# yoshitomo-matsubara/sc2-benchmark

Hardware: AMD Instinct MI355X
Metric: images/s + bpp, Entropic-Student ResNet-50 224^2 (higher is better)
Workload: dtype bf16

## Files before the change

### sc2-benchmark_amd/csrc/conv1x1_kres.hip

```cpp
#include <stdlib.h>

#include <atomic>

#include <type_traits>

#include "sc2_common.h"

#ifndef SC2_NT_KRES
#define SC2_NT_KRES 0
#endif

namespace {

typedef __attribute__((address_space(3))) void *lds_ptr_t;
typedef float f32x2_t __attribute__((ext_vector_type(2)));
typedef __bf16 bf16x2_t __attribute__((ext_vector_type(2)));
__device__ __forceinline__ uint32_t pack2(f32x2_t v) {
    return __builtin_bit_cast(uint32_t, __builtin_convertvector(v, bf16x2_t));
}

#if defined(__HIP_DEVICE_COMPILE__)
typedef __amdgpu_buffer_rsrc_t buf_rsrc_t;
__device__ __forceinline__ buf_rsrc_t make_rsrc(const uint16_t *base, uint32_t bytes) {
    return __builtin_amdgcn_make_buffer_rsrc(const_cast<uint16_t *>(base), 0, (int)bytes, 0x00020000);
}
__device__ __forceinline__ void buf_load_lds16(buf_rsrc_t r, lds_ptr_t dst, uint32_t voff, uint32_t soff) {
    __builtin_amdgcn_raw_ptr_buffer_load_lds(r, dst, 16, (int)voff, (int)soff, 0, 0);
}
#else
typedef int buf_rsrc_t;
__device__ __forceinline__ buf_rsrc_t make_rsrc(const uint16_t *, uint32_t) { return 0; }
__device__ __forceinline__ void buf_load_lds16(buf_rsrc_t, lds_ptr_t, uint32_t, uint32_t) {}
#endif

__device__ __forceinline__ uint4 lds_read16(uint32_t addr) {
    uint4 v;
    asm volatile("ds_read_b128 %0, %1" : "=v"(v) : "v"(addr) : "memory");
    return v;
}

struct KresArgs {
    const uint16_t *__restrict__ x;
    const uint16_t *__restrict__ w;
    const float *__restrict__ bias;
    uint16_t *__restrict__ y;
    int M, Cout, relu, n_chunks, n_tiles;
    int H, W, OW, OHW, stride;
    unsigned in_bytes;
    unsigned *unit_ctr;
};

template <int K_, int BM_, int BNC_>
struct KresShape {
    static constexpr int K = K_, BM = BM_, BNC = BNC_;
    static constexpr int KS = K / 32, KSH = KS / 2;
    static constexpr int MT = BM / 16, NTW = BNC / 32;
    static constexpr int NB = MT * NTW, NOWN = NB / 2;
    static constexpr int A_BYTES = BM * K * 2;
    static constexpr int PPR = K * 2 / 1024;
    static constexpr int PIECES = A_BYTES / 1024, PIECES_PER_WAVE = PIECES / 4;
    static constexpr int XCH_OFF = 2 * A_BYTES;
    static constexpr int OIMG_OFF = XCH_OFF;
    static constexpr int LDS_BYTES = XCH_OFF + 16 * 1024;
    static constexpr int OUT_CHUNKS = BM * BNC * 2 / 16;
    static constexpr int STORES = OUT_CHUNKS >= 256 ? OUT_CHUNKS / 256 : 1;
    static_assert(A_BYTES == 65536 && (K / 64) * (BNC / 32) * 4 == 256, "64 KB A tile, 256 weight registers per wave");
    static_assert(4 * NOWN * 1024 <= 16 * 1024 && BM * BNC * 2 <= 16 * 1024 && STORES >= 1, "exchange / image area");
    static_assert(LDS_BYTES + 64 <= 160 * 1024, "one workgroup per CU");
};

template <class S>
__global__ __launch_bounds__(256, 1) void conv1x1_kres_kernel(const KresArgs p) {
    constexpr int K = S::K, BM = S::BM, BNC = S::BNC, KS = S::KS, KSH = S::KSH, MT = S::MT, NTW = S::NTW, NOWN = S::NOWN;
    extern __shared__ __attribute__((aligned(16))) unsigned char smem[];
    __shared__ int next_slot;
    const uint32_t lds_base = (uint32_t)(uintptr_t)(lds_ptr_t)smem;
    const int tid = threadIdx.x;
    const int lane = tid & 63;
    const int wave = __builtin_amdgcn_readfirstlane(tid >> 6);
    const int kh = wave >> 1, nh = wave & 1;
    const int frow = lane & 15, fq = lane >> 4;

    const int xcd = blockIdx.x & 7;
    const int j_x = blockIdx.x >> 3;
    const int chunk = j_x % p.n_chunks;
    const int wg_l = j_x / p.n_chunks;
    const int wgs_x = ((int)gridDim.x - xcd + 7) >> 3;
    const int wgs_c = (wgs_x - chunk + p.n_chunks - 1) / p.n_chunks;
    const int n_local = (p.n_tiles - xcd + 7) >> 3;
    unsigned *const my_ctr = p.unit_ctr + xcd * 16 + chunk;

    uint4 wreg[KSH][NTW];
    {
        const uint4 *wf = reinterpret_cast<const uint4 *>(p.w) + lane;
#pragma unroll
        for (int j = 0; j < NTW; ++j)
#pragma unroll
            for (int s = 0; s < KSH; ++s)
                wreg[s][j] = wf[((long long)(chunk * (BNC / 16) + nh * NTW + j) * KS + kh * KSH + s) * 64];
    }

    const buf_rsrc_t rs = make_rsrc(p.x, p.in_bytes);
    auto row_offsets = [&](int tile) -> uint32_t {
        const int m = (xcd + 8 * tile) * BM + (lane & (BM - 1));
        const bool ok = tile < n_local && m < p.M;
        long long pix = m;
        if (p.stride == 2) {
            const int mm = ok ? m : 0;
            const int im = mm / p.OHW, rem = mm - im * p.OHW;
            const int oh = rem / p.OW, ow = rem - oh * p.OW;
            pix = ((long long)im * p.H + 2 * oh) * p.W + 2 * ow;
        }
        return ok ? (uint32_t)(pix * (K * 2)) : 0xFFFFFFFFu;
    };
    auto issue_piece = [&](uint32_t rowoff_v, int buf, int k) {
        const int pc = wave + 4 * k;
        const int row = pc / S::PPR, part = pc % S::PPR;
        const uint32_t ro = (uint32_t)__builtin_amdgcn_readlane((int)rowoff_v, row);
        const bool ok = ro != 0xFFFFFFFFu;
        const uint32_t vo = ok ? (uint32_t)(((64 * part + lane) ^ (row & 15)) * 16) : 0x80000000u;
        buf_load_lds16(rs, (lds_ptr_t)(smem + buf * S::A_BYTES + pc * 1024), vo, ok ? ro : 0u);
    };

    int unit = wg_l;
    int next_unit = unit + wgs_c;
    {
        const uint32_t ro = row_offsets(unit);
#pragma unroll
        for (int k = 0; k < S::PIECES_PER_WAVE; ++k) issue_piece(ro, 0, k);
    }
    int g = 0;

    while (unit < n_local) {
        const int m0 = (xcd + 8 * unit) * BM;
        if (g != 0) asm volatile("s_waitcnt vmcnt(%0)" ::"n"(S::STORES) : "memory");
        else asm volatile("s_waitcnt vmcnt(0)" ::: "memory");
        __syncthreads();
        unsigned claimed = 0;
        if (tid == 0) {
            const unsigned one = 1u;
            asm volatile("global_atomic_add %0, %1, %2, off sc0" : "=v"(claimed) : "v"(my_ctr), "v"(one) : "memory");
        }
        const uint32_t ro_next = row_offsets(next_unit);
        const uint32_t ab = lds_base + (uint32_t)((g & 1) * S::A_BYTES);
        const uint32_t a_lane = ab + (uint32_t)(frow * (K * 2));
        f32x4_t acc[MT][NTW];
#pragma unroll
        for (int i = 0; i < MT; ++i)
#pragma unroll
            for (int j = 0; j < NTW; ++j) acc[i][j] = f32x4_t{0.f, 0.f, 0.f, 0.f};
        uint4 av[2][MT];
        {
            int fqo = fq;
            asm volatile("" : "+v"(fqo));
            const int ks = kh * KSH;
#pragma unroll
            for (int i = 0; i < MT; ++i)
                av[0][i] = lds_read16(a_lane + (uint32_t)(i * 16 * K * 2) + (uint32_t)((((ks * 4 + fqo) ^ frow)) << 4));
        }
        constexpr int PIECE_STEPS = 8;
        constexpr int PER_STEP = S::PIECES_PER_WAVE / PIECE_STEPS;
#pragma unroll
        for (int s = 0; s < KSH; ++s) {
            asm volatile("s_waitcnt lgkmcnt(0)" ::: "memory");
            __builtin_amdgcn_sched_barrier(0);
            if (s + 1 < KSH) {
                int fqo = fq;
                asm volatile("" : "+v"(fqo));
                const int ks = kh * KSH + s + 1;
#pragma unroll
                for (int i = 0; i < MT; ++i)
                    av[(s + 1) & 1][i] = lds_read16(a_lane + (uint32_t)(i * 16 * K * 2) + (uint32_t)((((ks * 4 + fqo) ^ frow)) << 4));
            }
#pragma unroll
            for (int i = 0; i < MT; ++i) {
                const bf16x8_t af = __builtin_bit_cast(bf16x8_t, av[s & 1][i]);
#pragma unroll
                for (int j = 0; j < NTW; ++j)
                    acc[i][j] = __builtin_amdgcn_mfma_f32_16x16x32_bf16(__builtin_bit_cast(bf16x8_t, wreg[s][j]), af, acc[i][j], 0, 0, 0);
            }
            __builtin_amdgcn_sched_barrier(0);
            if (s < PIECE_STEPS) {
#pragma unroll
                for (int q = 0; q < PER_STEP; ++q) issue_piece(ro_next, (g + 1) & 1, PER_STEP * s + q);
            }
        }
#pragma unroll
        for (int b = 0; b < NOWN; ++b) {
            const f32x4_t v = kh ? acc[b / NTW][b % NTW] : acc[(NOWN + b) / NTW][(NOWN + b) % NTW];
            *reinterpret_cast<f32x4_t *>(smem + S::XCH_OFF + ((wave * NOWN + b) * 64 + lane) * 16) = v;
        }
        __syncthreads();
        f32x4_t own[NOWN];
#pragma unroll
        for (int b = 0; b < NOWN; ++b) {
            const f32x4_t mine = kh ? acc[(NOWN + b) / NTW][(NOWN + b) % NTW] : acc[b / NTW][b % NTW];
            own[b] = mine + *reinterpret_cast<const f32x4_t *>(smem + S::XCH_OFF + (((wave ^ 2) * NOWN + b) * 64 + lane) * 16);
        }
        __syncthreads();
        {
            unsigned char *oimg = smem + S::OIMG_OFF;
            constexpr int CPI = BNC / 8;
            auto finish = [&](auto relu_c) {
                constexpr bool RELU = decltype(relu_c)::value;
#pragma unroll
                for (int b = 0; b < NOWN; ++b) {
                    const int bb = kh * NOWN + b;
                    const int i = bb / NTW, j = bb % NTW;
                    const int px = i * 16 + frow;
                    const int ch = nh * (BNC / 2) + j * 16 + fq * 4;
                    const float4 bias4 = *reinterpret_cast<const float4 *>(p.bias + chunk * BNC + ch);
                    f32x2_t v01 = f32x2_t{own[b][0], own[b][1]} + f32x2_t{bias4.x, bias4.y};
                    f32x2_t v23 = f32x2_t{own[b][2], own[b][3]} + f32x2_t{bias4.z, bias4.w};
                    if (RELU) {
                        v01 = f32x2_t{fmaxf(v01[0], 0.f), fmaxf(v01[1], 0.f)};
                        v23 = f32x2_t{fmaxf(v23[0], 0.f), fmaxf(v23[1], 0.f)};
                    }
                    uint2 o;
                    o.x = pack2(v01);
                    o.y = pack2(v23);
                    const int c = ch >> 3;
                    *reinterpret_cast<uint2 *>(oimg + px * (BNC * 2) + ((c ^ (px & (CPI - 1))) << 4) + (ch & 7) * 2) = o;
                }
            };
            if (p.relu) finish(std::true_type{});
            else finish(std::false_type{});
        }
        __syncthreads();
        {
            const unsigned char *oimg = smem + S::OIMG_OFF;
            uint4 *yo = reinterpret_cast<uint4 *>(p.y + (long long)chunk * BNC);
            constexpr int CPI = BNC / 8;
#pragma unroll
            for (int k = 0; k < S::STORES; ++k) {
                const int q = (tid + 256 * k) % S::OUT_CHUNKS;
                int row = q / CPI;
                const int c = q % CPI;
                row = m0 + row < p.M ? row : 0;
                const uint4 ov = *reinterpret_cast<const uint4 *>(oimg + row * (BNC * 2) + ((c ^ (row & (CPI - 1))) << 4));
                if (SC2_NT_KRES) sc2_store16_nt(yo + (long long)(m0 + row) * (p.Cout / 8) + c, ov);
                else yo[(long long)(m0 + row) * (p.Cout / 8) + c] = ov;
            }
        }
        if (tid == 0) {
            asm volatile("s_waitcnt vmcnt(%1)" : "+v"(claimed) : "n"(S::STORES) : "memory");
            next_slot = (int)(claimed + 2 * wgs_c);
            if (claimed == (unsigned)(n_local - 1)) *my_ctr = 0u;
        }
        __syncthreads();
        ++g;
        unit = next_unit;
        next_unit = __builtin_amdgcn_readfirstlane(next_slot);
    }
    asm volatile("s_waitcnt vmcnt(0)" ::: "memory");
}

constexpr int kRingK = 1024;
sc2_counter_ring g_ring_k;
std::atomic<unsigned> g_seq_k{0};

template <class S>
int launch_kres(KresArgs a, hipStream_t s) {
    a.n_chunks = a.Cout / S::BNC;
    a.n_tiles = (a.M + S::BM - 1) / S::BM;
    static bool attr_set_dev[SC2_MAX_DEVICES] = {};
    bool &attr_set = attr_set_dev[sc2_device_slot()];
    if (!attr_set) {
        (void)hipFuncSetAttribute(reinterpret_cast<const void *>(&conv1x1_kres_kernel<S>), hipFuncAttributeMaxDynamicSharedMemorySize,
                                  S::LDS_BYTES);
        attr_set = true;
    }
    const int g_cus_k = sc2_device_cus();
    unsigned *slot = g_ring_k.launch_slot(s, kRingK, 128, g_seq_k);
    if (!slot) return SC2_ERR_INTERNAL;
    const long long units = (long long)a.n_tiles * a.n_chunks;
    int grid = units < g_cus_k ? (int)units : g_cus_k;
    if (grid < 8 * a.n_chunks) grid = 8 * a.n_chunks;
    a.unit_ctr = slot;
    hipLaunchKernelGGL(conv1x1_kres_kernel<S>, dim3(grid), dim3(256), S::LDS_BYTES, s, a);
    SC2_CHECK_LAUNCH();
    return SC2_OK;
}

}

extern "C" int sc2_conv1x1_kres_supported(int Cin, int Cout, int stride) {
    if (stride != 1 && stride != 2) return 0;
    if (Cin == 1024) return Cout >= 128 && Cout % 128 == 0 && Cout <= 16 * 128 ? 1 : 0;
    if (Cin == 2048) return Cout >= 64 && Cout % 64 == 0 && Cout <= 16 * 64 ? 1 : 0;
    return 0;
}

extern "C" int sc2_conv1x1_kres_fwd(const void *x, const void *w_frag, const float *bias, void *y, int N, int H, int W, int Cin,
                                    int Cout, int stride, int relu, void *stream) {
    SC2_REQUIRE(x && w_frag && bias && y, SC2_ERR_INVALID_ARG, "conv1x1_kres: null argument");
    SC2_REQUIRE(N > 0 && H > 0 && W > 0, SC2_ERR_INVALID_ARG, "conv1x1_kres: non-positive dimension");
    SC2_REQUIRE(sc2_conv1x1_kres_supported(Cin, Cout, stride), SC2_ERR_UNSUPPORTED,
                "conv1x1_kres: needs Cin 1024 (Cout %% 128 == 0, <= 2048) or 2048 (Cout %% 64 == 0, <= 1024), stride 1 or 2 "
                "(got %d -> %d, stride %d)", Cin, Cout, stride);
    const long long in_bytes = (long long)N * H * W * Cin * 2;
    SC2_REQUIRE(in_bytes < 0x7FF00000LL, SC2_ERR_UNSUPPORTED, "conv1x1_kres: input of %lld bytes exceeds 2 GB", in_bytes);
    KresArgs a;
    a.x = static_cast<const uint16_t *>(x);
    a.w = static_cast<const uint16_t *>(w_frag);
    a.bias = bias;
    a.y = static_cast<uint16_t *>(y);
    a.H = H; a.W = W; a.stride = stride;
    const int OH = (H - 1) / stride + 1;
    a.OW = (W - 1) / stride + 1;
    a.OHW = OH * a.OW;
    a.M = N * a.OHW; a.Cout = Cout; a.relu = relu ? 1 : 0;
    a.in_bytes = (unsigned)in_bytes;
    a.n_chunks = 0; a.n_tiles = 0; a.unit_ctr = nullptr;
    hipStream_t s = static_cast<hipStream_t>(stream);
    if (Cin == 1024) return launch_kres<KresShape<1024, 32, 128>>(a, s);
    return launch_kres<KresShape<2048, 16, 64>>(a, s);
}
```

Baseline: 44760.

## Cut workgroup barriers in 1x1 conv epilogue and spread next-tile prefetch

Reworks the per-unit epilogue of the persistent 1x1 conv kernel. The exchange and output-image areas now get separate LDS regions, which removes one barrier, and the next-unit slot is passed through LDS so the final barrier disappears. Bias is moved into registers once per workgroup, and the next-tile row offsets are computed inside the first k-step. Prefetch pieces are spread over 16 k-steps instead of 8. An optional timestamp probe is also added behind a compile flag. The changes aim to shorten epilogue serialization, at the cost of extra LDS and registers and subtle hazards from the reduced synchronization.

```diff
diff --git a/sc2-benchmark_amd/csrc/conv1x1_kres.hip b/sc2-benchmark_amd/csrc/conv1x1_kres.hip
--- a/sc2-benchmark_amd/csrc/conv1x1_kres.hip
+++ b/sc2-benchmark_amd/csrc/conv1x1_kres.hip
@@ -1,3 +1,4 @@
+#include <stdio.h>
 #include <stdlib.h>
 
 #include <atomic>
@@ -38,6 +39,43 @@
     asm volatile("ds_read_b128 %0, %1" : "=v"(v) : "v"(addr) : "memory");
     return v;
 }
+typedef unsigned u32x4_t __attribute__((ext_vector_type(4)));
+typedef unsigned u32x2_t __attribute__((ext_vector_type(2)));
+__device__ __forceinline__ void lds_write16(uint32_t addr, u32x4_t q) { asm volatile("ds_write_b128 %0, %1" ::"v"(addr), "v"(q) : "memory"); }
+__device__ __forceinline__ void lds_write8(uint32_t addr, u32x2_t q) { asm volatile("ds_write_b64 %0, %1" ::"v"(addr), "v"(q) : "memory"); }
+__device__ __forceinline__ void lds_write4(uint32_t addr, uint32_t v) { asm volatile("ds_write_b32 %0, %1" ::"v"(addr), "v"(v) : "memory"); }
+__device__ __forceinline__ uint32_t lds_read4(uint32_t addr) {
+    uint32_t v;
+    asm volatile("ds_read_b32 %0, %1" : "=v"(v) : "v"(addr) : "memory");
+    return v;
+}
+__device__ __forceinline__ void lds_wait() {
+    asm volatile("s_waitcnt lgkmcnt(0)" ::: "memory");
+    __builtin_amdgcn_sched_barrier(0);
+}
+__device__ __forceinline__ void wg_barrier() {
+    asm volatile("s_waitcnt lgkmcnt(0)" ::: "memory");
+    __builtin_amdgcn_s_barrier();
+    __builtin_amdgcn_sched_barrier(0);
+}
+
+#ifndef SC2_KRES_STAMPS
+#define SC2_KRES_STAMPS 0
+#endif
+#if SC2_KRES_STAMPS
+constexpr int N_STAMP = 8;
+constexpr int STAMP_BYTES = 4 * 16 * N_STAMP * 8;
+#define KSTAMP(k)                                                                                                         \
+    do {                                                                                                                  \
+        if (lane == 0 && g < 16) {                                                                                        \
+            const unsigned long long t_ = __builtin_amdgcn_s_memtime();                                                   \
+            asm volatile("ds_write_b64 %0, %1" ::"v"(stamp_base + (uint32_t)((g * N_STAMP + (k)) * 8)), "v"(t_) : "memory"); \
+        }                                                                                                                 \
+    } while (0)
+#else
+constexpr int STAMP_BYTES = 0;
+#define KSTAMP(k) do { } while (0)
+#endif
 
 struct KresArgs {
     const uint16_t *__restrict__ x;
@@ -48,6 +86,7 @@
     int H, W, OW, OHW, stride;
     unsigned in_bytes;
     unsigned *unit_ctr;
+    unsigned long long *stamps;
 };
 
 template <int K_, int BM_, int BNC_>
@@ -60,26 +99,37 @@
     static constexpr int PPR = K * 2 / 1024;
     static constexpr int PIECES = A_BYTES / 1024, PIECES_PER_WAVE = PIECES / 4;
     static constexpr int XCH_OFF = 2 * A_BYTES;
-    static constexpr int OIMG_OFF = XCH_OFF;
-    static constexpr int LDS_BYTES = XCH_OFF + 16 * 1024;
+    static constexpr int OIMG_OFF = XCH_OFF + 16 * 1024;
+    static constexpr int CTL_OFF = OIMG_OFF + 8 * 1024;
+    static constexpr int LDS_BYTES = CTL_OFF + 64;
     static constexpr int OUT_CHUNKS = BM * BNC * 2 / 16;
     static constexpr int STORES = OUT_CHUNKS >= 256 ? OUT_CHUNKS / 256 : 1;
     static_assert(A_BYTES == 65536 && (K / 64) * (BNC / 32) * 4 == 256, "64 KB A tile, 256 weight registers per wave");
-    static_assert(4 * NOWN * 1024 <= 16 * 1024 && BM * BNC * 2 <= 16 * 1024 && STORES >= 1, "exchange / image area");
-    static_assert(LDS_BYTES + 64 <= 160 * 1024, "one workgroup per CU");
+    static_assert(4 * NOWN * 1024 <= 16 * 1024 && BM * BNC * 2 <= 8 * 1024 && STORES >= 1, "exchange / image area");
+    static_assert(PIECES_PER_WAVE <= KSH, "one piece of the next unit behind a k-step");
+    static_assert(LDS_BYTES + STAMP_BYTES + 64 <= 160 * 1024, "one workgroup per CU");
 };
+
+#ifndef SC2_KRES_PIECE_STEPS
+#define SC2_KRES_PIECE_STEPS 16
+#endif
 
 template <class S>
 __global__ __launch_bounds__(256, 1) void conv1x1_kres_kernel(const KresArgs p) {
     constexpr int K = S::K, BM = S::BM, BNC = S::BNC, KS = S::KS, KSH = S::KSH, MT = S::MT, NTW = S::NTW, NOWN = S::NOWN;
     extern __shared__ __attribute__((aligned(16))) unsigned char smem[];
-    __shared__ int next_slot;
     const uint32_t lds_base = (uint32_t)(uintptr_t)(lds_ptr_t)smem;
     const int tid = threadIdx.x;
     const int lane = tid & 63;
     const int wave = __builtin_amdgcn_readfirstlane(tid >> 6);
     const int kh = wave >> 1, nh = wave & 1;
     const int frow = lane & 15, fq = lane >> 4;
+    const uint32_t next_slot_addr = lds_base + (uint32_t)S::CTL_OFF;
+#if SC2_KRES_STAMPS
+    const uint32_t stamp_base = lds_base + (uint32_t)(S::LDS_BYTES + wave * (16 * N_STAMP * 8));
+    for (int k = tid; k < STAMP_BYTES / 8; k += 256) *reinterpret_cast<unsigned long long *>(smem + S::LDS_BYTES + k * 8) = 0ull;
+    __syncthreads();
+#endif
 
     const int xcd = blockIdx.x & 7;
     const int j_x = blockIdx.x >> 3;
@@ -98,6 +148,12 @@
 #pragma unroll
             for (int s = 0; s < KSH; ++s)
                 wreg[s][j] = wf[((long long)(chunk * (BNC / 16) + nh * NTW + j) * KS + kh * KSH + s) * 64];
+    }
+    float4 breg[NOWN];
+#pragma unroll
+    for (int b = 0; b < NOWN; ++b) {
+        const int j = (kh * NOWN + b) % NTW;
+        breg[b] = *reinterpret_cast<const float4 *>(p.bias + chunk * BNC + nh * (BNC / 2) + j * 16 + fq * 4);
     }
 
     const buf_rsrc_t rs = make_rsrc(p.x, p.in_bytes);
@@ -131,17 +187,23 @@
     }
     int g = 0;
 
+    const uint32_t xch_w = lds_base + (uint32_t)(S::XCH_OFF + (wave * NOWN * 64 + lane) * 16);
+    const uint32_t xch_r = lds_base + (uint32_t)(S::XCH_OFF + ((wave ^ 2) * NOWN * 64 + lane) * 16);
+    const uint32_t oimg = lds_base + (uint32_t)S::OIMG_OFF;
+
     while (unit < n_local) {
         const int m0 = (xcd + 8 * unit) * BM;
+        KSTAMP(0);
         if (g != 0) asm volatile("s_waitcnt vmcnt(%0)" ::"n"(S::STORES) : "memory");
         else asm volatile("s_waitcnt vmcnt(0)" ::: "memory");
-        __syncthreads();
+        wg_barrier();
+        KSTAMP(1);
         unsigned claimed = 0;
         if (tid == 0) {
             const unsigned one = 1u;
             asm volatile("global_atomic_add %0, %1, %2, off sc0" : "=v"(claimed) : "v"(my_ctr), "v"(one) : "memory");
         }
-        const uint32_t ro_next = row_offsets(next_unit);
+        uint32_t ro_next = 0;
         const uint32_t ab = lds_base + (uint32_t)((g & 1) * S::A_BYTES);
         const uint32_t a_lane = ab + (uint32_t)(frow * (K * 2));
         f32x4_t acc[MT][NTW];
@@ -158,8 +220,9 @@
             for (int i = 0; i < MT; ++i)
                 av[0][i] = lds_read16(a_lane + (uint32_t)(i * 16 * K * 2) + (uint32_t)((((ks * 4 + fqo) ^ frow)) << 4));
         }
-        constexpr int PIECE_STEPS = 8;
+        constexpr int PIECE_STEPS = SC2_KRES_PIECE_STEPS;
         constexpr int PER_STEP = S::PIECES_PER_WAVE / PIECE_STEPS;
+        static_assert(PER_STEP * PIECE_STEPS == S::PIECES_PER_WAVE && PIECE_STEPS <= KSH, "pieces per k-step");
 #pragma unroll
         for (int s = 0; s < KSH; ++s) {
             asm volatile("s_waitcnt lgkmcnt(0)" ::: "memory");
@@ -172,6 +235,7 @@
                 for (int i = 0; i < MT; ++i)
                     av[(s + 1) & 1][i] = lds_read16(a_lane + (uint32_t)(i * 16 * K * 2) + (uint32_t)((((ks * 4 + fqo) ^ frow)) << 4));
             }
+            if (s == 0) ro_next = row_offsets(next_unit);
 #pragma unroll
             for (int i = 0; i < MT; ++i) {
                 const bf16x8_t af = __builtin_bit_cast(bf16x8_t, av[s & 1][i]);
@@ -184,75 +248,89 @@
 #pragma unroll
                 for (int q = 0; q < PER_STEP; ++q) issue_piece(ro_next, (g + 1) & 1, PER_STEP * s + q);
             }
+            if (s == KSH / 2 - 1) KSTAMP(2);
+        }
+        KSTAMP(3);
+        asm volatile("s_waitcnt vmcnt(%1)" : "+v"(claimed) : "n"(S::PIECES_PER_WAVE) : "memory");
+        if (tid == 0) {
+            lds_write4(next_slot_addr, claimed + 2u * (unsigned)wgs_c);
+            if (claimed == (unsigned)(n_local - 1)) *my_ctr = 0u;
         }
 #pragma unroll
         for (int b = 0; b < NOWN; ++b) {
             const f32x4_t v = kh ? acc[b / NTW][b % NTW] : acc[(NOWN + b) / NTW][(NOWN + b) % NTW];
-            *reinterpret_cast<f32x4_t *>(smem + S::XCH_OFF + ((wave * NOWN + b) * 64 + lane) * 16) = v;
-        }
-        __syncthreads();
-        f32x4_t own[NOWN];
-#pragma unroll
-        for (int b = 0; b < NOWN; ++b) {
-            const f32x4_t mine = kh ? acc[(NOWN + b) / NTW][(NOWN + b) % NTW] : acc[b / NTW][b % NTW];
-            own[b] = mine + *reinterpret_cast<const f32x4_t *>(smem + S::XCH_OFF + (((wave ^ 2) * NOWN + b) * 64 + lane) * 16);
-        }
-        __syncthreads();
+            lds_write16(xch_w + (uint32_t)(b * 1024), __builtin_bit_cast(u32x4_t, v));
+        }
+        wg_barrier();
+        KSTAMP(4);
+        uint4 part[NOWN];
+#pragma unroll
+        for (int b = 0; b < NOWN; ++b) part[b] = lds_read16(xch_r + (uint32_t)(b * 1024));
+        const uint32_t ns = lds_read4(next_slot_addr);
+        lds_wait();
         {
-            unsigned char *oimg = smem + S::OIMG_OFF;
             constexpr int CPI = BNC / 8;
             auto finish = [&](auto relu_c) {
                 constexpr bool RELU = decltype(relu_c)::value;
 #pragma unroll
                 for (int b = 0; b < NOWN; ++b) {
+                    const f32x4_t mine = kh ? acc[(NOWN + b) / NTW][(NOWN + b) % NTW] : acc[b / NTW][b % NTW];
+                    const f32x4_t own = mine + __builtin_bit_cast(f32x4_t, part[b]);
                     const int bb = kh * NOWN + b;
                     const int i = bb / NTW, j = bb % NTW;
                     const int px = i * 16 + frow;
                     const int ch = nh * (BNC / 2) + j * 16 + fq * 4;
-                    const float4 bias4 = *reinterpret_cast<const float4 *>(p.bias + chunk * BNC + ch);
-                    f32x2_t v01 = f32x2_t{own[b][0], own[b][1]} + f32x2_t{bias4.x, bias4.y};
-                    f32x2_t v23 = f32x2_t{own[b][2], own[b][3]} + f32x2_t{bias4.z, bias4.w};
+                    const float4 bias4 = breg[b];
+                    f32x2_t v01 = f32x2_t{own[0], own[1]} + f32x2_t{bias4.x, bias4.y};
+                    f32x2_t v23 = f32x2_t{own[2], own[3]} + f32x2_t{bias4.z, bias4.w};
                     if (RELU) {
                         v01 = f32x2_t{fmaxf(v01[0], 0.f), fmaxf(v01[1], 0.f)};
                         v23 = f32x2_t{fmaxf(v23[0], 0.f), fmaxf(v23[1], 0.f)};
                     }
-                    uint2 o;
-                    o.x = pack2(v01);
-                    o.y = pack2(v23);
+                    const u32x2_t o = {pack2(v01), pack2(v23)};
                     const int c = ch >> 3;
-                    *reinterpret_cast<uint2 *>(oimg + px * (BNC * 2) + ((c ^ (px & (CPI - 1))) << 4) + (ch & 7) * 2) = o;
+                    lds_write8(oimg + (uint32_t)(px * (BNC * 2) + ((c ^ (px & (CPI - 1))) << 4) + (ch & 7) * 2), o);
                 }
             };
             if (p.relu) finish(std::true_type{});
             else finish(std::false_type{});
         }
-        __syncthreads();
+        wg_barrier();
+        KSTAMP(5);
         {
-            const unsigned char *oimg = smem + S::OIMG_OFF;
             uint4 *yo = reinterpret_cast<uint4 *>(p.y + (long long)chunk * BNC);
             constexpr int CPI = BNC / 8;
+            uint4 ov[S::STORES];
+            int orow[S::STORES], oc[S::STORES];
 #pragma unroll
             for (int k = 0; k < S::STORES; ++k) {
                 const int q = (tid + 256 * k) % S::OUT_CHUNKS;
                 int row = q / CPI;
                 const int c = q % CPI;
                 row = m0 + row < p.M ? row : 0;
-                const uint4 ov = *reinterpret_cast<const uint4 *>(oimg + row * (BNC * 2) + ((c ^ (row & (CPI - 1))) << 4));
-                if (SC2_NT_KRES) sc2_store16_nt(yo + (long long)(m0 + row) * (p.Cout / 8) + c, ov);
-                else yo[(long long)(m0 + row) * (p.Cout / 8) + c] = ov;
+                orow[k] = row;
+                oc[k] = c;
+                ov[k] = lds_read16(oimg + (uint32_t)(row * (BNC * 2) + ((c ^ (row & (CPI - 1))) << 4)));
             }
-        }
-        if (tid == 0) {
-            asm volatile("s_waitcnt vmcnt(%1)" : "+v"(claimed) : "n"(S::STORES) : "memory");
-            next_slot = (int)(claimed + 2 * wgs_c);
-            if (claimed == (unsigned)(n_local - 1)) *my_ctr = 0u;
-        }
-        __syncthreads();
+            lds_wait();
+#pragma unroll
+            for (int k = 0; k < S::STORES; ++k) {
+                if (SC2_NT_KRES) sc2_store16_nt(yo + (long long)(m0 + orow[k]) * (p.Cout / 8) + oc[k], ov[k]);
+                else yo[(long long)(m0 + orow[k]) * (p.Cout / 8) + oc[k]] = ov[k];
+            }
+        }
+        KSTAMP(6);
         ++g;
         unit = next_unit;
-        next_unit = __builtin_amdgcn_readfirstlane(next_slot);
+        next_unit = __builtin_amdgcn_readfirstlane((int)ns);
     }
     asm volatile("s_waitcnt vmcnt(0)" ::: "memory");
+#if SC2_KRES_STAMPS
+    wg_barrier();
+    if (p.stamps && blockIdx.x < 8)
+        for (int k = tid; k < STAMP_BYTES / 8; k += 256)
+            p.stamps[blockIdx.x * (STAMP_BYTES / 8) + k] = *reinterpret_cast<const unsigned long long *>(smem + S::LDS_BYTES + k * 8);
+#endif
 }
 
 constexpr int kRingK = 1024;
@@ -267,7 +345,7 @@
     bool &attr_set = attr_set_dev[sc2_device_slot()];
     if (!attr_set) {
         (void)hipFuncSetAttribute(reinterpret_cast<const void *>(&conv1x1_kres_kernel<S>), hipFuncAttributeMaxDynamicSharedMemorySize,
-                                  S::LDS_BYTES);
+                                  S::LDS_BYTES + STAMP_BYTES);
         attr_set = true;
     }
     const int g_cus_k = sc2_device_cus();
@@ -277,8 +355,30 @@
     int grid = units < g_cus_k ? (int)units : g_cus_k;
     if (grid < 8 * a.n_chunks) grid = 8 * a.n_chunks;
     a.unit_ctr = slot;
-    hipLaunchKernelGGL(conv1x1_kres_kernel<S>, dim3(grid), dim3(256), S::LDS_BYTES, s, a);
+    a.stamps = nullptr;
+#if SC2_KRES_STAMPS
+    const char *stamp_path = getenv("SC2_KRES_STAMPS");
+    const size_t stamp_bytes = 8 * (size_t)STAMP_BYTES;
+    if (stamp_path) {
+        void *sp = nullptr;
+        (void)hipMalloc(&sp, stamp_bytes);
+        (void)hipMemset(sp, 0, stamp_bytes);
+        a.stamps = static_cast<unsigned long long *>(sp);
+    }
+#endif
+    hipLaunchKernelGGL(conv1x1_kres_kernel<S>, dim3(grid), dim3(256), S::LDS_BYTES + STAMP_BYTES, s, a);
     SC2_CHECK_LAUNCH();
+#if SC2_KRES_STAMPS
+    if (a.stamps) {
+        (void)hipStreamSynchronize(s);
+        unsigned long long *host = static_cast<unsigned long long *>(malloc(stamp_bytes));
+        (void)hipMemcpy(host, a.stamps, stamp_bytes, hipMemcpyDeviceToHost);
+        (void)hipFree(a.stamps);
+        FILE *f = fopen(stamp_path, "wb");
+        if (f) { fwrite(host, 1, stamp_bytes, f); fclose(f); }
+        free(host);
+    }
+#endif
     return SC2_OK;
 }
 
@@ -311,7 +411,7 @@
     a.OHW = OH * a.OW;
     a.M = N * a.OHW; a.Cout = Cout; a.relu = relu ? 1 : 0;
     a.in_bytes = (unsigned)in_bytes;
-    a.n_chunks = 0; a.n_tiles = 0; a.unit_ctr = nullptr;
+    a.n_chunks = 0; a.n_tiles = 0; a.unit_ctr = nullptr; a.stamps = nullptr;
     hipStream_t s = static_cast<hipStream_t>(stream);
     if (Cin == 1024) return launch_kres<KresShape<1024, 32, 128>>(a, s);
     return launch_kres<KresShape<2048, 16, 64>>(a, s);
```

After: 45110 (median of 6 runs). Within noise of the previous version (+0.8%).
